# yhwu/rsicnv

Hardware: AMD Instinct MI355X
Metric: bases/sec through RSI pipeline (bin+GC+NB+segment) (higher is better)
Workload: dtype int32

## Files before the change

### rsicnv_amd/csrc/kernels.h

```cpp
#pragma once
#include <hip/hip_runtime.h>
#include <stdint.h>
#include <mutex>
#include "device_util.h"

namespace rsik {

inline void note_launch() {
  const hipError_t e = hipGetLastError();
  if (e != hipSuccess && tl_launch_error == hipSuccess) tl_launch_error = e;
}
inline void drain_stale_errors() { (void)hipGetLastError(); tl_launch_error = hipSuccess; }
inline hipError_t take_launch_error() { const hipError_t e = tl_launch_error; tl_launch_error = hipSuccess; return e; }
#define RSI_LAUNCH(...) do { hipLaunchKernelGGL(__VA_ARGS__); rsik::note_launch(); } while (0)

constexpr int kGcLevels = 202;
constexpr int kHistValues = 65536;
constexpr int kResClasses = 32;
constexpr int kTileBases = 4096;

void launch_fasta_classify(const uint8_t* fasta, int64_t n, uint64_t* gcbits, uint64_t* nbits, int64_t nwords,
                           const FillList& fill, hipStream_t stream);
void launch_fill(const FillList& fill, hipStream_t stream);
size_t fold_scratch_bytes();
// ... 106 lines not shown
enum class K4Route { stream, joint, bytes, wide16, int32 };
struct K4Plan {
  K4Route route;
  bool fixed;
  bool raw;
  bool bytes_fit;
  ByteShape shape;
  const char* marks[2];
};
K4Plan k4_plan(bool gcadjust, bool capped, int32_t capval, int m, int64_t ncompact, int nreg, bool deep, bool joint_ok,
               const PerBaseSwitches& sw);

void launch_nb_raw(const int64_t* binsum, int64_t nb, int m, int64_t ncompact, double r, float* raw,
                   uint32_t* rawmin_bits, hipStream_t stream);
struct MinMaxF { uint32_t min_inv, max_bits; unsigned int nonfinite; unsigned int pad; };
struct GridMedian { double med, ymin; unsigned long long count; uint32_t np, flags; };
enum { kGridEmpty = 1, kGridNonFinite = 2, kGridDegenerate = 4, kGridTooWide = 8 };
struct GridChain { MinMaxF* mm; uint32_t* hist; uint32_t cap; unsigned int* counters; };
struct GridExport { const void* src[2]; void* dst[2]; size_t bytes[2]; };

void launch_nb_scale_minmax(float* x, int64_t nb, const uint32_t* rawmin_bits, double med_raw, double del_raw, double dup_raw,
                            double RDmedian, const GridChain& c, GridMedian* out, hipStream_t stream);
void launch_i32_to_f32_minmax(const int32_t* in, float* out_f, int64_t nb, double center, const GridChain& c, GridMedian* out,
                              hipStream_t stream);
void launch_minmax_f32(const float* x, const int32_t* mask, int64_t nb, int use_abs, double center, MinMaxF* mm,
                       hipStream_t stream);
void launch_hist_f32(const float* x, const int32_t* mask, int64_t nb, int use_abs, double center, double ymin,
                     uint32_t* hist, uint32_t np, hipStream_t stream);
void launch_minmax_plan(const float* x, const int32_t* mask, int64_t nb, int use_abs, double center, const double* d_center,
                        const GridChain& c, GridMedian* out, hipStream_t stream);
void launch_hist_walk(const float* x, const int32_t* mask, int64_t nb, int use_abs, double center, const double* d_center,
                      const GridChain& c, GridMedian* out, const GridExport* ex, const FillList* fill, hipStream_t stream);
bool hist_walk_pack16(int64_t nb);

struct ScanParams {
  int64_t nb;
  int32_t Lmax;
  int16_t pad;
  int16_t kcap;
  double tmedian;
  double lim_del;
  double lim_dup;
};
constexpr int kMaxScanL = 10400;
constexpr int kScanLdsL = 3800;
constexpr int kScanPad = 8;
constexpr int kThrInline = 232;
// ... 138 lines not shown
```

### rsicnv_amd/csrc/kernels_bin.hip

```cpp
#include <type_traits>
#include "kernels.h"
#include "device_util.h"

namespace rsik {

namespace {

constexpr int kThreads = 256;
constexpr int kMaxGrid = 256 * 2;

__device__ inline int lane_id() { return threadIdx.x & 63; }
inline int grid_for(int64_t items, int per_block) {
  int64_t g = (items + per_block - 1) / per_block;
  if (g < 1) g = 1;
  if (g > kMaxGrid) g = kMaxGrid;
  return (int)g;
}

__device__ inline uint32_t f32_key(float f) {
  const uint32_t b = __float_as_uint(f);
  return (b & 0x80000000u) ? ~b : (b | 0x80000000u);
}

__global__ __launch_bounds__(kThreads) void k_nb_raw(const int64_t* __restrict__ binsum, int64_t nb, int m,
// ... 51 lines not shown
    for (int w = 1; w < kThreads / 64; ++w) { kmin = s_min[w] < kmin ? s_min[w] : kmin; kmax = s_max[w] > kmax ? s_max[w] : kmax; bad |= s_bad[w]; }
    if (kmin != 0xffffffffu) atomicMax(&mm->min_inv, ~kmin);
    if (kmax != 0) atomicMax(&mm->max_bits, kmax);
    if (bad) atomicOr(&mm->nonfinite, 1u);
  }
}

__global__ __launch_bounds__(kThreads) void k_minmax_f32(const float* __restrict__ x, const int32_t* __restrict__ mask,
                                                         int64_t nb, int use_abs, double center, MinMaxF* __restrict__ mm) {
  minmax_body(x, mask, nb, use_abs, center, mm);
}
constexpr uint32_t kLdsBins = 12288;

constexpr int kHistRun = 8;

template <bool PACK16 = false>
__device__ __forceinline__ void hist_body(const float* __restrict__ x, const int32_t* __restrict__ mask, int64_t nb, int use_abs,
                                          double center, double ymin, uint32_t* __restrict__ hist, uint32_t np, int use_lds,
                                          unsigned int* s_h) {
  const uint32_t nl = use_lds ? (np < (uint32_t)use_lds ? np : (uint32_t)use_lds) : 0;
  auto lds_add = [&](uint32_t k, uint32_t c) { if (PACK16) atomicAdd(&s_h[k >> 1], c << ((k & 1u) << 4)); else atomicAdd(&s_h[k], c); };
  auto bucket = [&](float v) {
    const double idx = ((double)v - ymin) / 0.01 + 0.5;
    uint32_t k = (uint32_t)(unsigned long long)idx;
    return k >= np ? np - 1 : k;
  };
  __shared__ uint32_t s_wb;
  if (threadIdx.x == 0) s_wb = 0u;
  if (use_lds) { for (uint32_t e = threadIdx.x; e < (PACK16 ? (nl + 1) / 2 : nl); e += kThreads) s_h[e] = 0; }
  if (use_lds && np > nl && threadIdx.x < 64) {
    const int lane = (int)threadIdx.x;
    const int64_t i = (int64_t)(((unsigned long long)(2 * lane + 1) * (unsigned long long)nb) >> 7);
    const bool valid = i < nb && !(mask && mask[i] != 0);
    const uint32_t k = valid ? bucket(sel_value(x, i, use_abs, center)) : 0xffffffffu;
    int rank = 0;
    for (int j = 0; j < 64; ++j) {
      const uint32_t kj = (uint32_t)__builtin_amdgcn_readlane((int)k, j);
      rank += (kj < k || (kj == k && j < lane)) ? 1 : 0;
    }
    const int nvalid = __popcll(__ballot(valid));
    if (valid && rank == nvalid / 2) s_wb = k < nl / 2 ? 0u : (k - nl / 2 > np - nl ? np - nl : k - nl / 2);
  }
  if (use_lds) __syncthreads();
  const uint32_t wb = use_lds ? s_wb : 0u;
  auto count = [&](uint32_t k, uint32_t c) { if (k - wb < nl) lds_add(k - wb, c); else atomicAdd(&hist[k], c); };
  const int64_t nchunks = (nb + kHistRun - 1) / kHistRun;
  for (int64_t c = (int64_t)blockIdx.x * kThreads + threadIdx.x; c < nchunks; c += (int64_t)gridDim.x * kThreads) {
    uint32_t pend_k = 0xffffffffu, pend_c = 0;
    const int64_t i0 = c * kHistRun, i1 = i0 + kHistRun < nb ? i0 + kHistRun : nb;
    auto one = [&](float xv) {
      const float v = use_abs ? (float)fabs((double)xv - center) : xv;
      const uint32_t k = bucket(v);
      if (k != pend_k) {
        if (pend_c) count(pend_k, pend_c);
        pend_k = k; pend_c = 0;
      }
      ++pend_c;
    };
    if (i1 - i0 == kHistRun) {
      static_assert(kHistRun == 8, "two quads per run");
      const float4 a = *reinterpret_cast<const float4*>(x + i0), b = *reinterpret_cast<const float4*>(x + i0 + 4);
      int4 ma = make_int4(0, 0, 0, 0), mb = ma;
      if (mask) { ma = *reinterpret_cast<const int4*>(mask + i0); mb = *reinterpret_cast<const int4*>(mask + i0 + 4); }
      const float xv[8] = {a.x, a.y, a.z, a.w, b.x, b.y, b.z, b.w};
      const int mv[8] = {ma.x, ma.y, ma.z, ma.w, mb.x, mb.y, mb.z, mb.w};
#pragma unroll
      for (int e = 0; e < 8; ++e) if (mv[e] == 0) one(xv[e]);
    } else {
      for (int64_t i = i0; i < i1; ++i) {
        if (mask && mask[i] != 0) continue;
        one(x[i]);
      }
    }
    if (pend_c) count(pend_k, pend_c);
  }
  if (use_lds) {
    __syncthreads();
    for (uint32_t e = threadIdx.x; e < nl; e += kThreads) {
      const unsigned int c = PACK16 ? (s_h[e >> 1] >> ((e & 1u) << 4)) & 0xffffu : s_h[e];
      if (c) atomicAdd(&hist[wb + e], c);
    }
  }
}

__global__ __launch_bounds__(kThreads) void k_hist_f32(const float* __restrict__ x, const int32_t* __restrict__ mask,
                                                       int64_t nb, int use_abs, double center, double ymin,
                                                       uint32_t* __restrict__ hist, uint32_t np, int use_lds) {
  extern __shared__ unsigned int s_h[];
  hist_body(x, mask, nb, use_abs, center, ymin, hist, np, use_lds, s_h);
}

__device__ inline float f32_unkey(uint32_t k) { return __uint_as_float((k & 0x80000000u) ? (k & 0x7fffffffu) : ~k); }

__device__ inline void grid_plan_block(MinMaxF* __restrict__ mm, uint32_t cap, uint32_t* __restrict__ hist, GridMedian* __restrict__ g) {
  const uint32_t kmin = ~ld_cg(&mm->min_inv), kmax = ld_cg(&mm->max_bits), bad = ld_cg(&mm->nonfinite);
  uint32_t flags = 0, np = 0;
  double ymin = 0.0;
  if (kmin == 0xffffffffu) flags = kGridEmpty;
  else if (bad) flags = kGridNonFinite;
  else {
    ymin = (double)f32_unkey(kmin);
    const double ymax = (double)f32_unkey(kmax);
    if ((ymax - ymin) < 0.01) flags = kGridDegenerate;
    else {
      const size_t n = (size_t)((ymax - ymin) / 0.01 + 2);
      if (n > cap) flags = kGridTooWide; else np = (uint32_t)n;
    }
  }
  for (uint32_t e = threadIdx.x; e < np; e += kThreads) hist[e] = 0;
  __syncthreads();
  if (threadIdx.x == 0) {
    g->med = 0.0; g->ymin = ymin; g->count = 0; g->np = np; g->flags = flags;
    mm->min_inv = 0; mm->max_bits = 0; mm->nonfinite = 0;
  }
}

__device__ inline void minmax_commit(uint32_t kmin, uint32_t kmax, unsigned int bad, MinMaxF* __restrict__ mm) {
  for (int d = 32; d >= 1; d >>= 1) {
    const uint32_t a = __shfl_xor(kmin, d), b = __shfl_xor(kmax, d);
    kmin = a < kmin ? a : kmin; kmax = b > kmax ? b : kmax; bad |= __shfl_xor(bad, d);
  }
  __shared__ uint32_t s_min[kThreads / 64], s_max[kThreads / 64], s_bad[kThreads / 64];
  if (lane_id() == 0) { s_min[threadIdx.x >> 6] = kmin; s_max[threadIdx.x >> 6] = kmax; s_bad[threadIdx.x >> 6] = bad; }
  __syncthreads();
  if (threadIdx.x == 0) {
    for (int w = 1; w < kThreads / 64; ++w) { kmin = s_min[w] < kmin ? s_min[w] : kmin; kmax = s_max[w] > kmax ? s_max[w] : kmax; bad |= s_bad[w]; }
    if (kmin != 0xffffffffu) atomicMax(&mm->min_inv, ~kmin);
// ... 22 lines not shown
    float xv[4]; int mv[4] = {0, 0, 0, 0};
#pragma unroll
    for (int e = 0; e < 4; ++e) xv[e] = x[i + e * stride];
    if (mask) {
#pragma unroll
      for (int e = 0; e < 4; ++e) mv[e] = mask[i + e * stride];
    }
#pragma unroll
    for (int e = 0; e < 4; ++e) if (mv[e] == 0) one(xv[e]);
  }
  for (; i < nb; i += stride) {
    if (mask && mask[i] != 0) continue;
    one(x[i]);
  }
  minmax_commit(kmin, kmax, bad, mm);
  if (last_block_done(counter)) grid_plan_block(mm, cap, hist, g);
}

struct ExportPair { const void* src[2]; void* dst[2]; unsigned int bytes[2]; };

__device__ inline void grid_walk_block(const uint32_t* __restrict__ hist, GridMedian* __restrict__ g) {
  __shared__ unsigned long long s_sum[kThreads];
  __shared__ unsigned long long s_seen;
  __shared__ unsigned int s_cross;
  const uint32_t np = g->np;
  const uint32_t chunk = (((np + kThreads - 1) / kThreads) + 3u) & ~3u;
  const uint32_t b0 = threadIdx.x * chunk < np ? threadIdx.x * chunk : np;
  const uint32_t b1 = b0 + chunk < np ? b0 + chunk : np;
  const __amdgpu_buffer_rsrc_t rs = coherent_buffer(hist);
  unsigned long long mine = 0;
  for (uint32_t b = b0; b < b1; b += 32) {
    u32x4 v[8];
#pragma unroll
    for (int j = 0; j < 8; ++j) { const uint32_t q = b + 4u * j; v[j] = ld_cg_buf_x4(rs, (q < b1 ? q : b0) * 4u, 0u); }
#pragma unroll
    for (int j = 0; j < 8; ++j) {
      const uint32_t q = b + 4u * j;
      const unsigned int c[4] = {v[j].x, v[j].y, v[j].z, v[j].w};
#pragma unroll
      for (int e = 0; e < 4; ++e) mine += q + e < b1 ? c[e] : 0u;
    }
  }
  s_sum[threadIdx.x] = mine;
  if (threadIdx.x == 0) s_cross = 0xffffffffu;
  __syncthreads();
  unsigned long long seen = 0, total = 0;
  for (int t = 0; t < kThreads; ++t) { const unsigned long long v = s_sum[t]; if (t < (int)threadIdx.x) seen += v; total += v; }
  const unsigned long long r2 = total / 2;
  unsigned long long* med_bits = reinterpret_cast<unsigned long long*>(&g->med);
  if (threadIdx.x == 0) { st_cg(&g->count, total); if (r2 == 0) st_cg(med_bits, (unsigned long long)__double_as_longlong(g->ymin)); }
  if (r2 != 0 && mine != 0 && seen < r2 && seen + mine >= r2) { s_cross = b0; s_seen = seen; }
  __syncthreads();
  const uint32_t cb = s_cross;
  if (cb == 0xffffffffu) return;
  const unsigned long long before = s_seen;
  const uint32_t ce = cb + chunk < np ? cb + chunk : np;
  const uint32_t per = (chunk + kThreads - 1) / kThreads;
  const uint32_t m0 = cb + threadIdx.x * per < ce ? cb + threadIdx.x * per : ce;
  const uint32_t m1 = m0 + per < ce ? m0 + per : ce;
  unsigned long long part = 0;
  for (uint32_t bb = m0; bb < m1; ++bb) part += ld_cg(hist + bb);
  __syncthreads();
  s_sum[threadIdx.x] = part;
  __syncthreads();
  unsigned long long run = before;
  for (int t = 0; t < (int)threadIdx.x; ++t) run += s_sum[t];
  if (part != 0 && run < r2 && run + part >= r2) {
    for (uint32_t bb = m0; bb < m1; ++bb) {
      const unsigned long long upto = run + ld_cg(hist + bb);
      if (run < r2 && upto >= r2) st_cg(med_bits, (unsigned long long)__double_as_longlong(g->ymin + (double)bb * 0.01));
      run = upto;
    }
  }
}

template <bool PACK16>
__global__ __launch_bounds__(kThreads) void k_hist_walk(const float* __restrict__ x, const int32_t* __restrict__ mask,
                                                        int64_t nb, int use_abs, double center,
                                                        const double* __restrict__ center_ptr,
                                                        GridMedian* __restrict__ g, uint32_t* __restrict__ hist,
                                                        unsigned int* __restrict__ counter, ExportPair ex, FillList fill, uint32_t lds_bins) {
  extern __shared__ unsigned int s_h[];
  fill_ranges(fill);
  if (!g->flags) {
    const uint32_t np = g->np;
    hist_body<PACK16>(x, mask, nb, use_abs, center_ptr ? *center_ptr : center, g->ymin, hist, np, (int)lds_bins, s_h);
  }
  if (!last_block_done(counter)) return;
  if (!g->flags) grid_walk_block(hist, g);
  sync_drained();
  for (int k = 0; k < 2; ++k) export_words(ex.dst[k], ex.src[k], ex.bytes[k]);
}

struct NbLevels { double med_raw, del_raw, dup_raw, RDmedian; };
__global__ __launch_bounds__(kThreads) void k_nb_scale_mm(float* __restrict__ x, int64_t nb, const uint32_t* __restrict__ rawmin_inv,
                                                          NbLevels lv, MinMaxF* __restrict__ mm, unsigned int* __restrict__ counter,
                                                          uint32_t cap, uint32_t* __restrict__ hist, GridMedian* __restrict__ g) {
  const uint32_t key = ~(*rawmin_inv);
  const double tmin = (double)__uint_as_float((key & 0x80000000u) ? (key & 0x7fffffffu) : ~key);
  const double med_nbt = lv.med_raw - tmin;
  const double del_s = (lv.del_raw - tmin) / med_nbt * lv.RDmedian, dup_s = (lv.dup_raw - tmin) / med_nbt * lv.RDmedian;
  const double med_s = med_nbt / med_nbt * lv.RDmedian;
  const float lev0 = (float)del_s, lev1 = (float)dup_s, lev2 = (float)med_s;
  uint32_t kmin = 0xffffffffu, kmax = 0;
  unsigned int bad = 0;
  for (int64_t b = (int64_t)blockIdx.x * kThreads + threadIdx.x; b < nb; b += (int64_t)gridDim.x * kThreads) {
    float v = x[b];
    v = (float)((double)v - tmin);
    v = (float)((double)v / med_nbt * lv.RDmedian);
    if (b == 0) v = lev0;
    if (b == 1) v = lev1;
    if (b == 2) v = lev2;
    x[b] = v;
    if (!(fabsf(v) <= 3.0e38f)) bad = 1;
    const uint32_t k = f32_key(v);
    kmin = k < kmin ? k : kmin;
    kmax = k > kmax ? k : kmax;
  }
  minmax_commit(kmin, kmax, bad, mm);
  if (last_block_done(counter)) grid_plan_block(mm, cap, hist, g);
}

__global__ __launch_bounds__(kThreads) void k_i32_to_f32_mm(const int32_t* __restrict__ in, float* __restrict__ out, int64_t nb,
                                                            double center, MinMaxF* __restrict__ mm, unsigned int* __restrict__ counter,
                                                            uint32_t cap, uint32_t* __restrict__ hist, GridMedian* __restrict__ g) {
  uint32_t kmin = 0xffffffffu, kmax = 0;
  unsigned int bad = 0;
  for (int64_t b = (int64_t)blockIdx.x * kThreads + threadIdx.x; b < nb; b += (int64_t)gridDim.x * kThreads) {
    const float f = (float)in[b];
    out[b] = f;
    const float v = (float)fabs((double)f - center);
    if (!(fabsf(v) <= 3.0e38f)) bad = 1;
    const uint32_t k = f32_key(v);
    kmin = k < kmin ? k : kmin;
    kmax = k > kmax ? k : kmax;
  }
  minmax_commit(kmin, kmax, bad, mm);
  if (last_block_done(counter)) grid_plan_block(mm, cap, hist, g);
}

constexpr int kScanTile = 256;
constexpr uint32_t kUnmarked = 0xffffffffu;

template <class IX>
struct ScanLdsT {
  using index = IX;
  double* P;
  double* tot;
  uint32_t* TB;
  int* M;
  IX* CB;
  IX* RB;
  IX* PF;
// ... 712 lines not shown
  RSI_LAUNCH(k_hist_f32, dim3(grid), dim3(kThreads), lds, stream, x, mask, nb, use_abs, center, ymin, hist, np, use_lds);
}
void launch_minmax_plan(const float* x, const int32_t* mask, int64_t nb, int use_abs, double center, const double* d_center,
                        const GridChain& c, GridMedian* out, hipStream_t stream) {
  RSI_LAUNCH(k_minmax_plan, dim3(bounded_grid(nb, kThreads * 16, 256)), dim3(kThreads), 0, stream, x, mask, nb, use_abs, center, d_center, c.mm,
                     c.counters, c.cap, c.hist, out);
}
static int hist_walk_grid(int64_t nb) { const int g = grid_for(nb, kThreads * kHistRun * 2); return g > 256 ? 256 : g; }
bool hist_walk_pack16(int64_t nb) {
  const int64_t run = (int64_t)kThreads * kHistRun, stride = (int64_t)hist_walk_grid(nb) * run;
  const int64_t tail = nb % stride;
  const int64_t most = nb / stride * run + (tail < run ? tail : run);
  return most < 65536;
}
void launch_hist_walk(const float* x, const int32_t* mask, int64_t nb, int use_abs, double center, const double* d_center,
                      const GridChain& c, GridMedian* out, const GridExport* ex, const FillList* fill, hipStream_t stream) {
  const uint32_t bins = kLdsBins;
  const int grid = hist_walk_grid(nb);
  const bool pack16 = hist_walk_pack16(nb);
  const size_t lds = pack16 ? (size_t)bins * 2 : (size_t)bins * 4;
  ExportPair e{};
  if (ex) for (int k = 0; k < 2; ++k) { e.src[k] = ex->src[k]; e.dst[k] = ex->dst[k]; e.bytes[k] = (unsigned int)ex->bytes[k]; }
  FillList f{};
  if (fill) f = *fill;
  if (pack16) RSI_LAUNCH(k_hist_walk<true>, dim3(grid), dim3(kThreads), lds, stream, x, mask, nb, use_abs, center, d_center, out, c.hist, c.counters + 1, e, f, bins);
  else { RSI_ALLOW_FULL_LDS(k_hist_walk<false>); RSI_LAUNCH(k_hist_walk<false>, dim3(grid), dim3(kThreads), lds, stream, x, mask, nb, use_abs, center, d_center, out, c.hist, c.counters + 1, e, f, bins); }
}
constexpr int kGTileGrid = 256;
constexpr size_t kGTileBudget = size_t(8) << 30;
struct ScanShape { int count, kcap, grid; bool gtile, wide; size_t tile_bytes; };
static ScanShape scan_tile_shape(int Lmax) {
  ScanShape sh;
  const int halo = Lmax / 2 + 1;
  sh.count = kScanTile + 2 * halo;
  sh.kcap = 0;
  while ((2 << sh.kcap) <= Lmax && sh.kcap < 6) ++sh.kcap;
  sh.gtile = Lmax > kScanLdsL;
  sh.wide = Lmax > kScanNarrowL;
  if (!sh.gtile) while (sh.kcap > 0 && scan_lds_bytes(sh.count, sh.kcap) + 4 * kThreads * sizeof(int) + 1024 > 160 * 1024) --sh.kcap;
  sh.tile_bytes = scan_lds_bytes(sh.count, sh.kcap, sh.wide ? 4 : 2);
  sh.grid = kGTileGrid;
// ... 91 lines not shown
```

### rsicnv_amd/csrc/pipeline.hip

```cpp
#include <new>
#include "pipeline_internal.h"

using namespace rsik;
using namespace rsip;
using rsih::Candidate;
using rsih::Region;

namespace {

struct ScanPassOut { uint32_t escapes, inexact, ldel, ldup; };

struct ScanOut {
  double tmedian1 = 0, tsigma1 = 0, tlamda1 = 0, tmedian2 = 0, tsigma2 = 0, tlamda2 = 0;
  int Lmax = 0;
  rsih::IntSpan status2;
  std::vector<int> run_status;
  std::vector<rsih::IntSpan::Range> run_ranges;
  std::vector<Candidate> segs;
  uint32_t escapes = 0, inexact = 0;
  uint32_t tiles_listed = 0;
  std::vector<uint32_t> level_log[4];
  uint32_t stop_levels[4] = {0, 0, 0, 0};
  std::vector<std::string> fs_lines;
};
// ... 39 lines not shown
  if (np > (64u << 20)) return fail(ctx, RSI_ERR_UNSUPPORTED, "transformed bin range too wide for the 0.01 grid");
  HIPCHK(ctx->hist_f.ensure(np * 4));
  HIPCHK(hipMemsetAsync(ctx->hist_f.p, 0, np * 4, ctx->stream));
  { Timer t(ctx, "hist_f32"); launch_hist_f32(d_x, d_mask, nb, use_abs, center, ymin, ctx->hist_f.as<uint32_t>(), (uint32_t)np, ctx->stream); }
  std::vector<uint32_t> h(np);
  HIPCHK(copy_d2h(ctx, h.data(), ctx->hist_f.p, np * 4));
  HIPCHK(CTX_SYNC());
  uint64_t total = 0;
  for (uint32_t c : h) total += c;
  *count = total;
  *med = rsih::hist_median_grid(h.data(), np, total, ymin);
  return RSI_OK;
}

constexpr uint32_t kGridCap = 1u << 20;
constexpr int32_t kFsListCap = 1 << 20;
struct ChainOut { GridMedian g[2]; uint32_t rawmin_inv; uint32_t pad[15]; };
GridChain grid_chain(rsi_ctx* ctx) {
  uint8_t* small = ctx->small.as<uint8_t>();
  return GridChain{reinterpret_cast<MinMaxF*>(small + kOffMinMax), ctx->hist_f.as<uint32_t>(), kGridCap,
                   reinterpret_cast<unsigned int*>(small + kOffDone) + kDoneBinSlot};
}
void scan_fill_list(rsi_ctx* ctx, int pass, int64_t nb, FillList& fl) {
  uint8_t* small = ctx->small.as<uint8_t>();
  uint32_t* d_first_del = ctx->first_del.as<uint32_t>();
  const int64_t nbpad = (nb + 3) & ~int64_t(3);
  fill_add(fl, d_first_del, (size_t)(nbpad + nb) * 4, 0xffffffffu);
  fill_add(fl, small + kOffScanPass + (size_t)pass * kScanPassBytes, kScanPassBytes, 0u);
  fill_add(fl, small + kOffCounters, 32, 0u);
  if (pass == 0 && ctx->fs_ws.p) fill_add(fl, ctx->fs_ws.p, level_sums_head_bytes(kMaxL), 0u);
}
int grid_pair_issue(rsi_ctx* ctx, const float* d_x, const int32_t* d_mask, int64_t nb, bool with_median, double center, bool planned,
                    int fill_pass, ChainOut** out) {
  uint8_t* small = ctx->small.as<uint8_t>();
  GridMedian* d_g = reinterpret_cast<GridMedian*>(small + kOffGrid);
  const GridChain gc = grid_chain(ctx);
  ChainOut* slot = static_cast<ChainOut*>(mb_alloc(ctx, sizeof(ChainOut)));
  if (!slot) return fail(ctx, RSI_ERR_INTERNAL, "out of pinned mailbox memory");
  memset(slot, 0, sizeof(*slot));
  GateShared gs(ctx);
  if (with_median) {
    if (!planned) { Timer t(ctx, "minmax_plan"); launch_minmax_plan(d_x, d_mask, nb, 0, 0.0, nullptr, gc, d_g, ctx->stream); }
    { Timer t(ctx, "hist_walk"); launch_hist_walk(d_x, d_mask, nb, 0, 0.0, nullptr, gc, d_g, nullptr, nullptr, ctx->stream); }
    planned = false;
  }
  const double* d_center = with_median ? &d_g->med : nullptr;
  if (!planned) { Timer t(ctx, "minmax_plan"); launch_minmax_plan(d_x, d_mask, nb, 1, center, d_center, gc, d_g + 1, ctx->stream); }
  GridExport ex{};
  ex.src[0] = d_g; ex.dst[0] = slot->g; ex.bytes[0] = 2 * sizeof(GridMedian);
  ex.src[1] = small + kOffRawMin; ex.dst[1] = &slot->rawmin_inv; ex.bytes[1] = 4;
  FillList fl{};
  if (fill_pass >= 0) scan_fill_list(ctx, fill_pass, nb, fl);
  { Timer t(ctx, "hist_walk"); launch_hist_walk(d_x, d_mask, nb, 1, center, d_center, gc, d_g + 1, &ex, &fl, ctx->stream); }
  *out = slot;
  return RSI_OK;
}
struct Selection { const float* d_x; const int32_t* d_mask; int64_t nb; int use_abs; double center; };
int grid_result(rsi_ctx* ctx, const GridMedian& g, const Selection& sel, double* med, uint64_t* count) {
  if (g.flags & kGridEmpty) { *count = 0; *med = 0; return RSI_OK; }
  if (g.flags & kGridNonFinite) return fail(ctx, RSI_ERR_UNSUPPORTED, "non-finite value in the transformed bins");
  if (g.flags & kGridDegenerate) return selection_mean(ctx, sel.d_x, sel.d_mask, sel.nb, sel.use_abs, sel.center, med, count);
  *med = g.med; *count = g.count;
  return RSI_OK;
}

void scan_thresholds(double tmedian, double tlamda, int Lmax, std::vector<double>& del, std::vector<double>& dup) {
  del.assign((size_t)Lmax + 1 + kScanPad, -INFINITY);
  dup.assign((size_t)Lmax + 1 + kScanPad, INFINITY);
  del[0] = -1.0;
// ... 310 lines not shown
  { Timer t(ctx, "resolve_runs"); launch_resolve_runs(d_first_del, d_first_dup, work + 2, nb, d_status, d_copy, ctx->runs.as<uint64_t>(), d_count, kMaxRunEntries, d_done + 3, rslot, kEagerBounds, ctx->stream); }
  *work_slot = wslot; *runs_slot = rslot;
  return RSI_OK;
}

int run_scan(rsi_ctx* ctx, const rsi_params& P, bool use_med, const float* d_T, int64_t nb, double RDmedian,
             double factor, int LmaxBase, ChainOut* first, double nb_med_raw, double nb_del_raw, double nb_dup_raw, ScanOut& out) {
  const int32_t* d_medint = ctx->binmed.as<int32_t>();
  double tmedian, tsigma, tlamda, target, dev, absmed;
  uint64_t cnt;
  int rc, cal_max;
  float t0 = 0, t2 = 0;
  {
    Phase ph(ctx, "scan.quantiles");
    HIPCHK(CTX_SYNC());
    const GridMedian* g = first->g;
    if ((!use_med && (g[0].flags & kGridTooWide)) || (g[1].flags & kGridTooWide)) {
      GateShared gs(ctx);
      if (!use_med) {
        if ((rc = grid_median(ctx, d_T, nullptr, nb, 0, 0.0, &tmedian, &cnt)) != RSI_OK) return rc;
      } else {
        tmedian = RDmedian;
      }
      if ((rc = grid_median(ctx, d_T, nullptr, nb, 1, tmedian, &absmed, &cnt)) != RSI_OK) return rc;
    } else {
      tmedian = RDmedian;
      if (!use_med && (rc = grid_result(ctx, g[0], Selection{d_T, nullptr, nb, 0, 0.0}, &tmedian, &cnt)) != RSI_OK) return rc;
      if (!use_med && (g[0].flags & kGridDegenerate)) rc = grid_median(ctx, d_T, nullptr, nb, 1, tmedian, &absmed, &cnt);
      else rc = grid_result(ctx, g[1], Selection{d_T, nullptr, nb, 1, tmedian}, &absmed, &cnt);
      if (rc != RSI_OK) return rc;
// ... 124 lines not shown
          RunArgs ra;
          if ((rc = prepare_runs(ctx, runs, ra)) != RSI_OK) return rc;
          Timer t(ctx, "trim_runs");
          launch_trim_runs(d_T, d_st1f, ra.d_start, ra.d_end, ra.use_inl ? &ra.inl : nullptr, (int)runs.size(), (double)m0 - dev, (double)m0 + dev, ctx->stream);
        }
      }
    }
  }
  ph_filter.stop();
  Phase ph_q2(ctx, "scan.quantiles");
  double tmed2;
  uint64_t k = 0;
  ChainOut* second = nullptr;
  if ((rc = grid_pair_issue(ctx, d_T, d_st1f, nb, true, 0.0, false, 1, &second)) != RSI_OK) return rc;
  HIPCHK(CTX_SYNC());
  const GridMedian* g2 = second->g;
  {
    GateShared gs_q2(ctx);
    const bool wide2 = (g2[0].flags & kGridTooWide) != 0;
    if ((rc = wide2 ? grid_median(ctx, d_T, d_st1f, nb, 0, 0.0, &tmed2, &k) : grid_result(ctx, g2[0], Selection{d_T, d_st1f, nb, 0, 0.0}, &tmed2, &k)) != RSI_OK) return rc;
    if (k > (uint64_t)(nb / 2)) {
      tmedian = tmed2;
      if ((rc = (wide2 || (g2[1].flags & (kGridTooWide)) || (g2[0].flags & kGridDegenerate)) ? grid_median(ctx, d_T, d_st1f, nb, 1, tmedian, &absmed, &cnt)
                                                        : grid_result(ctx, g2[1], Selection{d_T, d_st1f, nb, 1, tmedian}, &absmed, &cnt)) != RSI_OK) return rc;
      tsigma = absmed / 0.6745;
      tlamda = factor * tsigma;
      tlamda = std::max(tlamda, target);
    }
  }
  out.tmedian2 = tmedian; out.tsigma2 = tsigma; out.tlamda2 = tlamda;
// ... 593 lines not shown
    const double r = RDmedian / mad;
    S.nb_mad = mad; S.nb_r = r;
    const double factor = sqrt(2.0 * (1.0 + P.epsilon) * log(3.1E9));
    const int LmaxBase = std::max(20, 10000 / P.m);

    HIPCHK(ctx->first_del.ensure((size_t)(2 * nb + 8) * 4));
    HIPCHK(ctx->status1.ensure((size_t)nb * 4));
    HIPCHK(ctx->status1f.ensure((size_t)nb * 4));
    HIPCHK(ctx->status2.ensure((size_t)nb * 4));
    HIPCHK(ctx->runs.ensure((size_t)kMaxRunEntries * 8));
    HIPCHK(ctx->scan_tiles.ensure((size_t)(nb / 256 + 2) * 4));
    HIPCHK(ctx->fs_ws.ensure(level_sums_workspace_bytes(nb, kFsListCap, kMaxL)));
    HIPCHK(ctx->fs_out.ensure((size_t)(2 * kMaxL + 1) * 8 + 64));

    HIPCHK(ctx->tnb.ensure((size_t)nb * 4));
    HIPCHK(ctx->hist_f.ensure((size_t)kGridCap * 4));
    uint32_t* d_rawmin = reinterpret_cast<uint32_t*>(small + kOffRawMin);
    GridMedian* d_g = reinterpret_cast<GridMedian*>(small + kOffGrid);
    { Timer t(ctx, "nb_raw"); launch_nb_raw(ctx->binsum.as<int64_t>(), nb, P.m, ncompact, r, ctx->tnb.as<float>(), d_rawmin, st); }
    auto nbf = [&](double sum) {
      const double mm = (double)P.m;
      return 2.0 * sqrt(r) * log(sqrt((sum + 0.25) / (mm * r - 0.5)) + sqrt(1.0 + (sum + 0.25) / (mm * r - 0.5)));
    };
    const double med_raw = nbf(RDmedian * P.m), del_raw = nbf(RDmedian / 2.0 * (double)P.m), dup_raw = nbf(RDmedian * 1.5 * (double)P.m);
    { Timer t(ctx, "nb_scale"); launch_nb_scale_minmax(ctx->tnb.as<float>(), nb, d_rawmin, med_raw, del_raw, dup_raw, RDmedian, grid_chain(ctx), d_g, st); }
    bool nb_planned = true;
    ctx->have_nb = true;

    ph_nb.stop();
    gs_nb.release();
    rsih::CallerInput in;
// ... 147 lines not shown
    double tot = 0;
    for (const KernelTime& k : ctx->ktimes) { float ms = 0; (void)hipEventElapsedTime(&ms, k.a, k.b); tot += ms; }
    S.t_kernels_ms = tot;
  }
  return RSI_OK;
}

int grid_debug_enter(rsi_ctx* ctx, int64_t nb, double* out, int32_t* info) {
  if (!ctx || !out || !info || nb <= 0 || nb >= (1ll << 31) - 4096) return fail(ctx, RSI_ERR_BAD_ARG, "bad argument");
  HIPCHK(hipSetDevice(ctx->device));
  if (!ctx_enter(ctx)) return RSI_ERR_HIP;
  mailbox_reset(ctx);
  const bool fresh = ctx->small.p == nullptr;
  HIPCHK(ctx->small.ensure(kSmallBytes));
  if (fresh) HIPCHK(hipMemsetAsync(ctx->small.p, 0, kHeaderBytes, ctx->stream));
  HIPCHK(ctx->hist_f.ensure((size_t)kGridCap * 4));
  for (int k = 0; k < 4; ++k) out[k] = 0.0;
  for (int k = 0; k < 8; ++k) info[k] = 0;
  info[0] = info[2] = info[4] = -1;
  return RSI_OK;
}
void grid_debug_record(const GridMedian& g, int32_t* info) { info[0] = (int32_t)g.flags; info[1] = (int32_t)g.np; }
int grid_debug_mad(rsi_ctx* ctx, const float* d_x, const int32_t* d_mask, int64_t nb, double center, bool planned, double* out,
                   int32_t* info) {
  ChainOut* co = nullptr;
  int rc;
  if ((rc = grid_pair_issue(ctx, d_x, d_mask, nb, false, center, planned, -1, &co)) != RSI_OK) return rc;
  HIPCHK(CTX_SYNC());
  const GridMedian g = co->g[1];
  grid_debug_record(g, info + 2);
  info[4] = hist_walk_pack16(nb) ? 1 : 0;
// ... 279 lines not shown
    HIPCHK(hipMemcpyAsync(ctx->status1f.p, mask, (size_t)nb * 4, hipMemcpyHostToDevice, ctx->stream));
    d_mask = ctx->status1f.as<int32_t>();
  }
  const float* d_x = ctx->tnb.as<float>();
  if (mode == 1) return grid_debug_mad(ctx, d_x, d_mask, nb, center, false, out, info);
  double med = 0, mad = 0;
  uint64_t c0 = 0, c1 = 0;
  if (mode == 2) {
    info[5] = 2;
    if ((rc = grid_median(ctx, d_x, d_mask, nb, 0, 0.0, &med, &c0)) != RSI_OK) return rc;
    if ((rc = grid_median(ctx, d_x, d_mask, nb, 1, med, &mad, &c1)) != RSI_OK) return rc;
  } else {
    ChainOut* co = nullptr;
    if ((rc = grid_pair_issue(ctx, d_x, d_mask, nb, true, 0.0, false, -1, &co)) != RSI_OK) return rc;
    HIPCHK(CTX_SYNC());
    const GridMedian g0 = co->g[0], g1 = co->g[1];
    grid_debug_record(g0, info);
    grid_debug_record(g1, info + 2);
    info[4] = hist_walk_pack16(nb) ? 1 : 0;
    if ((g0.flags | g1.flags) & kGridTooWide) {
      info[5] = 2;
      if ((rc = grid_median(ctx, d_x, d_mask, nb, 0, 0.0, &med, &c0)) != RSI_OK) return rc;
      if ((rc = grid_median(ctx, d_x, d_mask, nb, 1, med, &mad, &c1)) != RSI_OK) return rc;
    } else {
      if ((rc = grid_result(ctx, g0, Selection{d_x, d_mask, nb, 0, 0.0}, &med, &c0)) != RSI_OK) return rc;
      if (g0.flags & kGridDegenerate) { info[5] = 1; rc = grid_median(ctx, d_x, d_mask, nb, 1, med, &mad, &c1); }
      else rc = grid_result(ctx, g1, Selection{d_x, d_mask, nb, 1, med}, &mad, &c1);
      if (rc != RSI_OK) return rc;
    }
  }
// ... 140 lines not shown
```

Baseline: 214.5 billion.

## Plan MAD histogram speculatively during median histogram pass to skip minmax pass

Measured after the change: 216.0 billion (median of 6 runs). No clear change (+0.7%).

```diff
diff --git a/rsicnv_amd/csrc/kernels.h b/rsicnv_amd/csrc/kernels.h
--- a/rsicnv_amd/csrc/kernels.h
+++ b/rsicnv_amd/csrc/kernels.h
@@ -144,8 +144,9 @@
 void launch_nb_raw(const int64_t* binsum, int64_t nb, int m, int64_t ncompact, double r, float* raw,
                    uint32_t* rawmin_bits, hipStream_t stream);
 struct MinMaxF { uint32_t min_inv, max_bits; unsigned int nonfinite; unsigned int pad; };
-struct GridMedian { double med, ymin; unsigned long long count; uint32_t np, flags; };
-enum { kGridEmpty = 1, kGridNonFinite = 2, kGridDegenerate = 4, kGridTooWide = 8 };
+struct GridMedian { double med, ymin; unsigned long long count; uint32_t np, flags; uint32_t max_key, pad; };
+enum { kGridEmpty = 1, kGridNonFinite = 2, kGridDegenerate = 4, kGridTooWide = 8, kGridUnplanned = 16 };
+constexpr uint32_t kGridDevWin = 1024;
 struct GridChain { MinMaxF* mm; uint32_t* hist; uint32_t cap; unsigned int* counters; };
 struct GridExport { const void* src[2]; void* dst[2]; size_t bytes[2]; };
 
@@ -160,7 +161,8 @@
 void launch_minmax_plan(const float* x, const int32_t* mask, int64_t nb, int use_abs, double center, const double* d_center,
                         const GridChain& c, GridMedian* out, hipStream_t stream);
 void launch_hist_walk(const float* x, const int32_t* mask, int64_t nb, int use_abs, double center, const double* d_center,
-                      const GridChain& c, GridMedian* out, const GridExport* ex, const FillList* fill, hipStream_t stream);
+                      const GridChain& c, GridMedian* out, const GridExport* ex, const FillList* fill, hipStream_t stream,
+                      bool plan_mad = false);
 bool hist_walk_pack16(int64_t nb);
 
 struct ScanParams {
diff --git a/rsicnv_amd/csrc/kernels_bin.hip b/rsicnv_amd/csrc/kernels_bin.hip
--- a/rsicnv_amd/csrc/kernels_bin.hip
+++ b/rsicnv_amd/csrc/kernels_bin.hip
@@ -89,10 +89,10 @@
 
 constexpr int kHistRun = 8;
 
-template <bool PACK16 = false>
-__device__ __forceinline__ void hist_body(const float* __restrict__ x, const int32_t* __restrict__ mask, int64_t nb, int use_abs,
-                                          double center, double ymin, uint32_t* __restrict__ hist, uint32_t np, int use_lds,
-                                          unsigned int* s_h) {
+template <bool PACK16 = false, bool TRACK = false>
+__device__ __forceinline__ uint32_t hist_body(const float* __restrict__ x, const int32_t* __restrict__ mask, int64_t nb, int use_abs,
+                                              double center, double ymin, uint32_t* __restrict__ hist, uint32_t np, int use_lds,
+                                              unsigned int* s_h, unsigned int* s_d = nullptr, uint32_t* __restrict__ devwin = nullptr) {
   const uint32_t nl = use_lds ? (np < (uint32_t)use_lds ? np : (uint32_t)use_lds) : 0;
   auto lds_add = [&](uint32_t k, uint32_t c) { if (PACK16) atomicAdd(&s_h[k >> 1], c << ((k & 1u) << 4)); else atomicAdd(&s_h[k], c); };
   auto bucket = [&](float v) {
@@ -100,10 +100,11 @@
     uint32_t k = (uint32_t)(unsigned long long)idx;
     return k >= np ? np - 1 : k;
   };
-  __shared__ uint32_t s_wb;
-  if (threadIdx.x == 0) s_wb = 0u;
+  __shared__ uint32_t s_wb, s_db;
+  if (threadIdx.x == 0) { s_wb = 0u; s_db = 0u; }
   if (use_lds) { for (uint32_t e = threadIdx.x; e < (PACK16 ? (nl + 1) / 2 : nl); e += kThreads) s_h[e] = 0; }
-  if (use_lds && np > nl && threadIdx.x < 64) {
+  if (TRACK) { for (uint32_t e = threadIdx.x; e < kGridDevWin; e += kThreads) s_d[e] = 0; }
+  if (((use_lds && np > nl) || (TRACK && np > kGridDevWin)) && threadIdx.x < 64) {
     const int lane = (int)threadIdx.x;
     const int64_t i = (int64_t)(((unsigned long long)(2 * lane + 1) * (unsigned long long)nb) >> 7);
     const bool valid = i < nb && !(mask && mask[i] != 0);
@@ -114,23 +115,32 @@
       rank += (kj < k || (kj == k && j < lane)) ? 1 : 0;
     }
     const int nvalid = __popcll(__ballot(valid));
-    if (valid && rank == nvalid / 2) s_wb = k < nl / 2 ? 0u : (k - nl / 2 > np - nl ? np - nl : k - nl / 2);
-  }
-  if (use_lds) __syncthreads();
+    if (valid && rank == nvalid / 2) {
+      if (use_lds && np > nl) s_wb = k < nl / 2 ? 0u : (k - nl / 2 > np - nl ? np - nl : k - nl / 2);
+      if (TRACK && np > kGridDevWin) s_db = k < kGridDevWin / 2 ? 0u : (k - kGridDevWin / 2 > np - kGridDevWin ? np - kGridDevWin : k - kGridDevWin / 2);
+    }
+  }
+  if (use_lds || TRACK) __syncthreads();
   const uint32_t wb = use_lds ? s_wb : 0u;
+  const uint32_t db = TRACK ? s_db : 0u;
   auto count = [&](uint32_t k, uint32_t c) { if (k - wb < nl) lds_add(k - wb, c); else atomicAdd(&hist[k], c); };
+  auto closest = [&](uint32_t k, uint32_t dkey) { if (k - db < kGridDevWin) atomicMax(&s_d[k - db], ~dkey); };
   const int64_t nchunks = (nb + kHistRun - 1) / kHistRun;
   for (int64_t c = (int64_t)blockIdx.x * kThreads + threadIdx.x; c < nchunks; c += (int64_t)gridDim.x * kThreads) {
-    uint32_t pend_k = 0xffffffffu, pend_c = 0;
+    uint32_t pend_k = 0xffffffffu, pend_c = 0, pend_d = 0xffffffffu;
     const int64_t i0 = c * kHistRun, i1 = i0 + kHistRun < nb ? i0 + kHistRun : nb;
     auto one = [&](float xv) {
       const float v = use_abs ? (float)fabs((double)xv - center) : xv;
       const uint32_t k = bucket(v);
       if (k != pend_k) {
-        if (pend_c) count(pend_k, pend_c);
-        pend_k = k; pend_c = 0;
+        if (pend_c) { count(pend_k, pend_c); if (TRACK) closest(pend_k, pend_d); }
+        pend_k = k; pend_c = 0; pend_d = 0xffffffffu;
       }
       ++pend_c;
+      if (TRACK) {
+        const uint32_t dkey = f32_key((float)fabs((double)v - (ymin + (double)k * 0.01)));
+        pend_d = dkey < pend_d ? dkey : pend_d;
+      }
     };
     if (i1 - i0 == kHistRun) {
       static_assert(kHistRun == 8, "two quads per run");
@@ -147,15 +157,19 @@
         one(x[i]);
       }
     }
-    if (pend_c) count(pend_k, pend_c);
-  }
+    if (pend_c) { count(pend_k, pend_c); if (TRACK) closest(pend_k, pend_d); }
+  }
+  if (use_lds || TRACK) __syncthreads();
   if (use_lds) {
-    __syncthreads();
     for (uint32_t e = threadIdx.x; e < nl; e += kThreads) {
       const unsigned int c = PACK16 ? (s_h[e >> 1] >> ((e & 1u) << 4)) & 0xffffu : s_h[e];
       if (c) atomicAdd(&hist[wb + e], c);
     }
   }
+  if (TRACK) {
+    for (uint32_t e = threadIdx.x; e < kGridDevWin; e += kThreads) { const unsigned int d = s_d[e]; if (d) atomicMax(&devwin[e], d); }
+  }
+  return db;
 }
 
 __global__ __launch_bounds__(kThreads) void k_hist_f32(const float* __restrict__ x, const int32_t* __restrict__ mask,
@@ -167,10 +181,8 @@
 
 __device__ inline float f32_unkey(uint32_t k) { return __uint_as_float((k & 0x80000000u) ? (k & 0x7fffffffu) : ~k); }
 
-__device__ inline void grid_plan_block(MinMaxF* __restrict__ mm, uint32_t cap, uint32_t* __restrict__ hist, GridMedian* __restrict__ g) {
-  const uint32_t kmin = ~ld_cg(&mm->min_inv), kmax = ld_cg(&mm->max_bits), bad = ld_cg(&mm->nonfinite);
-  uint32_t flags = 0, np = 0;
-  double ymin = 0.0;
+__device__ inline void grid_plan_tests(uint32_t kmin, uint32_t kmax, unsigned int bad, uint32_t cap, uint32_t& flags, uint32_t& np, double& ymin) {
+  flags = 0; np = 0; ymin = 0.0;
   if (kmin == 0xffffffffu) flags = kGridEmpty;
   else if (bad) flags = kGridNonFinite;
   else {
@@ -182,10 +194,19 @@
       if (n > cap) flags = kGridTooWide; else np = (uint32_t)n;
     }
   }
+}
+
+__device__ inline void grid_plan_block(MinMaxF* __restrict__ mm, uint32_t cap, uint32_t* __restrict__ hist, GridMedian* __restrict__ g,
+                                       bool clear_dev) {
+  const uint32_t kmin = ~ld_cg(&mm->min_inv), kmax = ld_cg(&mm->max_bits), bad = ld_cg(&mm->nonfinite);
+  uint32_t flags, np;
+  double ymin;
+  grid_plan_tests(kmin, kmax, bad, cap, flags, np, ymin);
   for (uint32_t e = threadIdx.x; e < np; e += kThreads) hist[e] = 0;
+  if (clear_dev) { for (uint32_t e = threadIdx.x; e < kGridDevWin; e += kThreads) hist[cap + e] = 0; }
   __syncthreads();
   if (threadIdx.x == 0) {
-    g->med = 0.0; g->ymin = ymin; g->count = 0; g->np = np; g->flags = flags;
+    g->med = 0.0; g->ymin = ymin; g->count = 0; g->np = np; g->flags = flags; g->max_key = kmax; g->pad = 0;
     mm->min_inv = 0; mm->max_bits = 0; mm->nonfinite = 0;
   }
 }
@@ -238,15 +259,15 @@
     one(x[i]);
   }
   minmax_commit(kmin, kmax, bad, mm);
-  if (last_block_done(counter)) grid_plan_block(mm, cap, hist, g);
+  if (last_block_done(counter)) grid_plan_block(mm, cap, hist, g, !use_abs);
 }
 
 struct ExportPair { const void* src[2]; void* dst[2]; unsigned int bytes[2]; };
 
-__device__ inline void grid_walk_block(const uint32_t* __restrict__ hist, GridMedian* __restrict__ g) {
+__device__ inline uint32_t grid_walk_block(const uint32_t* __restrict__ hist, GridMedian* __restrict__ g) {
   __shared__ unsigned long long s_sum[kThreads];
   __shared__ unsigned long long s_seen;
-  __shared__ unsigned int s_cross;
+  __shared__ unsigned int s_cross, s_bb;
   const uint32_t np = g->np;
   const uint32_t chunk = (((np + kThreads - 1) / kThreads) + 3u) & ~3u;
   const uint32_t b0 = threadIdx.x * chunk < np ? threadIdx.x * chunk : np;
@@ -266,7 +287,7 @@
     }
   }
   s_sum[threadIdx.x] = mine;
-  if (threadIdx.x == 0) s_cross = 0xffffffffu;
+  if (threadIdx.x == 0) { s_cross = 0xffffffffu; s_bb = 0xffffffffu; }
   __syncthreads();
   unsigned long long seen = 0, total = 0;
   for (int t = 0; t < kThreads; ++t) { const unsigned long long v = s_sum[t]; if (t < (int)threadIdx.x) seen += v; total += v; }
@@ -276,7 +297,7 @@
   if (r2 != 0 && mine != 0 && seen < r2 && seen + mine >= r2) { s_cross = b0; s_seen = seen; }
   __syncthreads();
   const uint32_t cb = s_cross;
-  if (cb == 0xffffffffu) return;
+  if (cb == 0xffffffffu) return cb;
   const unsigned long long before = s_seen;
   const uint32_t ce = cb + chunk < np ? cb + chunk : np;
   const uint32_t per = (chunk + kThreads - 1) / kThreads;
@@ -292,26 +313,57 @@
   if (part != 0 && run < r2 && run + part >= r2) {
     for (uint32_t bb = m0; bb < m1; ++bb) {
       const unsigned long long upto = run + ld_cg(hist + bb);
-      if (run < r2 && upto >= r2) st_cg(med_bits, (unsigned long long)__double_as_longlong(g->ymin + (double)bb * 0.01));
+      if (run < r2 && upto >= r2) { st_cg(med_bits, (unsigned long long)__double_as_longlong(g->ymin + (double)bb * 0.01)); s_bb = bb; }
       run = upto;
     }
   }
-}
-
-template <bool PACK16>
+  __syncthreads();
+  return s_bb;
+}
+
+__device__ inline void grid_plan_mad_block(const GridMedian* __restrict__ g0, uint32_t bb, uint32_t db, uint32_t cap,
+                                           uint32_t* __restrict__ hist, GridMedian* __restrict__ g1) {
+  uint32_t flags = kGridUnplanned, np = 0, kmax = 0;
+  double ymin = 0.0;
+  if (bb != 0xffffffffu && bb - db < kGridDevWin) {
+    const uint32_t inv = ld_cg(hist + cap + (bb - db));
+    if (inv) {
+      const double c = g0->ymin + (double)bb * 0.01;
+      const float xmin = (float)g0->ymin, xmax = f32_unkey(g0->max_key);
+      const float vmin = f32_unkey(~inv);
+      const float va = (float)fabs((double)xmin - c), vb = (float)fabs((double)xmax - c);
+      const float vmax = va > vb ? va : vb;
+      const double M = fmax(fabs((double)xmin), fabs((double)xmax));
+      if ((double)vmin <= 0.005 - (1e-9 + 0x1p-48 * (M + 1.0))) {
+        kmax = f32_key(vmax);
+        grid_plan_tests(f32_key(vmin), kmax, !(fabsf(vmax) <= 3.0e38f), cap, flags, np, ymin);
+      }
+    }
+  }
+  for (uint32_t e = threadIdx.x; e < np; e += kThreads) hist[e] = 0;
+  __syncthreads();
+  if (threadIdx.x == 0) { g1->med = 0.0; g1->ymin = ymin; g1->count = 0; g1->np = np; g1->flags = flags; g1->max_key = kmax; g1->pad = 0; }
+}
+
+template <bool PACK16, bool TRACK>
 __global__ __launch_bounds__(kThreads) void k_hist_walk(const float* __restrict__ x, const int32_t* __restrict__ mask,
                                                         int64_t nb, int use_abs, double center,
                                                         const double* __restrict__ center_ptr,
                                                         GridMedian* __restrict__ g, uint32_t* __restrict__ hist,
-                                                        unsigned int* __restrict__ counter, ExportPair ex, FillList fill, uint32_t lds_bins) {
+                                                        unsigned int* __restrict__ counter, ExportPair ex, FillList fill, uint32_t lds_bins,
+                                                        uint32_t cap) {
   extern __shared__ unsigned int s_h[];
   fill_ranges(fill);
+  uint32_t db = 0;
   if (!g->flags) {
     const uint32_t np = g->np;
-    hist_body<PACK16>(x, mask, nb, use_abs, center_ptr ? *center_ptr : center, g->ymin, hist, np, (int)lds_bins, s_h);
+    db = hist_body<PACK16, TRACK>(x, mask, nb, use_abs, center_ptr ? *center_ptr : center, g->ymin, hist, np, (int)lds_bins, s_h,
+                                  s_h + (PACK16 ? lds_bins / 2 : lds_bins), hist + cap);
   }
   if (!last_block_done(counter)) return;
-  if (!g->flags) grid_walk_block(hist, g);
+  uint32_t bb = 0xffffffffu;
+  if (!g->flags) bb = grid_walk_block(hist, g);
+  if (TRACK) grid_plan_mad_block(g, bb, db, cap, hist, g + 1);
   sync_drained();
   for (int k = 0; k < 2; ++k) export_words(ex.dst[k], ex.src[k], ex.bytes[k]);
 }
@@ -342,7 +394,7 @@
     kmax = k > kmax ? k : kmax;
   }
   minmax_commit(kmin, kmax, bad, mm);
-  if (last_block_done(counter)) grid_plan_block(mm, cap, hist, g);
+  if (last_block_done(counter)) grid_plan_block(mm, cap, hist, g, true);
 }
 
 __global__ __launch_bounds__(kThreads) void k_i32_to_f32_mm(const int32_t* __restrict__ in, float* __restrict__ out, int64_t nb,
@@ -360,7 +412,7 @@
     kmax = k > kmax ? k : kmax;
   }
   minmax_commit(kmin, kmax, bad, mm);
-  if (last_block_done(counter)) grid_plan_block(mm, cap, hist, g);
+  if (last_block_done(counter)) grid_plan_block(mm, cap, hist, g, false);
 }
 
 constexpr int kScanTile = 256;
@@ -1103,17 +1155,24 @@
   return most < 65536;
 }
 void launch_hist_walk(const float* x, const int32_t* mask, int64_t nb, int use_abs, double center, const double* d_center,
-                      const GridChain& c, GridMedian* out, const GridExport* ex, const FillList* fill, hipStream_t stream) {
+                      const GridChain& c, GridMedian* out, const GridExport* ex, const FillList* fill, hipStream_t stream, bool plan_mad) {
   const uint32_t bins = kLdsBins;
   const int grid = hist_walk_grid(nb);
   const bool pack16 = hist_walk_pack16(nb);
-  const size_t lds = pack16 ? (size_t)bins * 2 : (size_t)bins * 4;
+  const size_t lds = (pack16 ? (size_t)bins * 2 : (size_t)bins * 4) + (plan_mad ? (size_t)kGridDevWin * 4 : 0);
   ExportPair e{};
   if (ex) for (int k = 0; k < 2; ++k) { e.src[k] = ex->src[k]; e.dst[k] = ex->dst[k]; e.bytes[k] = (unsigned int)ex->bytes[k]; }
   FillList f{};
   if (fill) f = *fill;
-  if (pack16) RSI_LAUNCH(k_hist_walk<true>, dim3(grid), dim3(kThreads), lds, stream, x, mask, nb, use_abs, center, d_center, out, c.hist, c.counters + 1, e, f, bins);
-  else { RSI_ALLOW_FULL_LDS(k_hist_walk<false>); RSI_LAUNCH(k_hist_walk<false>, dim3(grid), dim3(kThreads), lds, stream, x, mask, nb, use_abs, center, d_center, out, c.hist, c.counters + 1, e, f, bins); }
+#define RSI_HIST_WALK(P16, TRK) RSI_LAUNCH((k_hist_walk<P16, TRK>), dim3(grid), dim3(kThreads), lds, stream, x, mask, nb, use_abs, center, d_center, out, c.hist, c.counters + 1, e, f, bins, c.cap)
+  if (plan_mad) {
+    if (pack16) RSI_HIST_WALK(true, true);
+    else { RSI_ALLOW_FULL_LDS((k_hist_walk<false, true>)); RSI_HIST_WALK(false, true); }
+  } else {
+    if (pack16) RSI_HIST_WALK(true, false);
+    else { RSI_ALLOW_FULL_LDS((k_hist_walk<false, false>)); RSI_HIST_WALK(false, false); }
+  }
+#undef RSI_HIST_WALK
 }
 constexpr int kGTileGrid = 256;
 constexpr size_t kGTileBudget = size_t(8) << 30;
diff --git a/rsicnv_amd/csrc/pipeline.hip b/rsicnv_amd/csrc/pipeline.hip
--- a/rsicnv_amd/csrc/pipeline.hip
+++ b/rsicnv_amd/csrc/pipeline.hip
@@ -77,6 +77,7 @@
 }
 
 constexpr uint32_t kGridCap = 1u << 20;
+constexpr size_t kGridHistBytes = ((size_t)kGridCap + kGridDevWin) * 4;
 constexpr int32_t kFsListCap = 1 << 20;
 struct ChainOut { GridMedian g[2]; uint32_t rawmin_inv; uint32_t pad[15]; };
 GridChain grid_chain(rsi_ctx* ctx) {
@@ -104,8 +105,8 @@
   GateShared gs(ctx);
   if (with_median) {
     if (!planned) { Timer t(ctx, "minmax_plan"); launch_minmax_plan(d_x, d_mask, nb, 0, 0.0, nullptr, gc, d_g, ctx->stream); }
-    { Timer t(ctx, "hist_walk"); launch_hist_walk(d_x, d_mask, nb, 0, 0.0, nullptr, gc, d_g, nullptr, nullptr, ctx->stream); }
-    planned = false;
+    { Timer t(ctx, "hist_walk"); launch_hist_walk(d_x, d_mask, nb, 0, 0.0, nullptr, gc, d_g, nullptr, nullptr, ctx->stream, true); }
+    planned = true;
   }
   const double* d_center = with_median ? &d_g->med : nullptr;
   if (!planned) { Timer t(ctx, "minmax_plan"); launch_minmax_plan(d_x, d_mask, nb, 1, center, d_center, gc, d_g + 1, ctx->stream); }
@@ -116,6 +117,25 @@
   if (fill_pass >= 0) scan_fill_list(ctx, fill_pass, nb, fl);
   { Timer t(ctx, "hist_walk"); launch_hist_walk(d_x, d_mask, nb, 1, center, d_center, gc, d_g + 1, &ex, &fl, ctx->stream); }
   *out = slot;
+  return RSI_OK;
+}
+void phase_count(rsi_ctx* ctx, const char* name) {
+  for (auto& p : ctx->phases) if (p.first == name) { p.second += 1.0; return; }
+  ctx->phases.push_back({name, 1.0});
+}
+int grid_pair_settle(rsi_ctx* ctx, const float* d_x, const int32_t* d_mask, int64_t nb, ChainOut* slot) {
+  if (!(slot->g[1].flags & kGridUnplanned)) { phase_count(ctx, "spec.madplan accepted"); return RSI_OK; }
+  phase_count(ctx, "spec.madplan rejected");
+  uint8_t* small = ctx->small.as<uint8_t>();
+  GridMedian* d_g = reinterpret_cast<GridMedian*>(small + kOffGrid);
+  const GridChain gc = grid_chain(ctx);
+  GateShared gs(ctx);
+  { Timer t(ctx, "minmax_plan"); launch_minmax_plan(d_x, d_mask, nb, 1, 0.0, &d_g->med, gc, d_g + 1, ctx->stream); }
+  GridExport ex{};
+  ex.src[0] = d_g; ex.dst[0] = slot->g; ex.bytes[0] = 2 * sizeof(GridMedian);
+  ex.src[1] = small + kOffRawMin; ex.dst[1] = &slot->rawmin_inv; ex.bytes[1] = 4;
+  { Timer t(ctx, "hist_walk"); launch_hist_walk(d_x, d_mask, nb, 1, 0.0, &d_g->med, gc, d_g + 1, &ex, nullptr, ctx->stream); }
+  HIPCHK(CTX_SYNC());
   return RSI_OK;
 }
 struct Selection { const float* d_x; const int32_t* d_mask; int64_t nb; int use_abs; double center; };
@@ -456,6 +476,7 @@
   {
     Phase ph(ctx, "scan.quantiles");
     HIPCHK(CTX_SYNC());
+    if (!use_med && (rc = grid_pair_settle(ctx, d_T, nullptr, nb, first)) != RSI_OK) return rc;
     const GridMedian* g = first->g;
     if ((!use_med && (g[0].flags & kGridTooWide)) || (g[1].flags & kGridTooWide)) {
       GateShared gs(ctx);
@@ -610,6 +631,7 @@
   ChainOut* second = nullptr;
   if ((rc = grid_pair_issue(ctx, d_T, d_st1f, nb, true, 0.0, false, 1, &second)) != RSI_OK) return rc;
   HIPCHK(CTX_SYNC());
+  if ((rc = grid_pair_settle(ctx, d_T, d_st1f, nb, second)) != RSI_OK) return rc;
   const GridMedian* g2 = second->g;
   {
     GateShared gs_q2(ctx);
@@ -1233,7 +1255,7 @@
     HIPCHK(ctx->fs_out.ensure((size_t)(2 * kMaxL + 1) * 8 + 64));
 
     HIPCHK(ctx->tnb.ensure((size_t)nb * 4));
-    HIPCHK(ctx->hist_f.ensure((size_t)kGridCap * 4));
+    HIPCHK(ctx->hist_f.ensure(kGridHistBytes));
     uint32_t* d_rawmin = reinterpret_cast<uint32_t*>(small + kOffRawMin);
     GridMedian* d_g = reinterpret_cast<GridMedian*>(small + kOffGrid);
     { Timer t(ctx, "nb_raw"); launch_nb_raw(ctx->binsum.as<int64_t>(), nb, P.m, ncompact, r, ctx->tnb.as<float>(), d_rawmin, st); }
@@ -1411,7 +1433,7 @@
   const bool fresh = ctx->small.p == nullptr;
   HIPCHK(ctx->small.ensure(kSmallBytes));
   if (fresh) HIPCHK(hipMemsetAsync(ctx->small.p, 0, kHeaderBytes, ctx->stream));
-  HIPCHK(ctx->hist_f.ensure((size_t)kGridCap * 4));
+  HIPCHK(ctx->hist_f.ensure(kGridHistBytes));
   for (int k = 0; k < 4; ++k) out[k] = 0.0;
   for (int k = 0; k < 8; ++k) info[k] = 0;
   info[0] = info[2] = info[4] = -1;
@@ -1721,6 +1743,7 @@
     ChainOut* co = nullptr;
     if ((rc = grid_pair_issue(ctx, d_x, d_mask, nb, true, 0.0, false, -1, &co)) != RSI_OK) return rc;
     HIPCHK(CTX_SYNC());
+    if ((rc = grid_pair_settle(ctx, d_x, d_mask, nb, co)) != RSI_OK) return rc;
     const GridMedian g0 = co->g[0], g1 = co->g[1];
     grid_debug_record(g0, info);
     grid_debug_record(g1, info + 2);
```
